# OpenDriveLab/ST-P3

Measured on AMD Instinct MI355X. Metric: BEV samples/sec (6-cam x 3-frame fwd+bwd), higher is better.
Workload: dtype bf16 convs / f32 voxel pool; 1 GPU; BASELINE configs[2]: batch=4/GPU, 6-cam 224x480, T=3, full STP3 fwd+bwd with segmentation + pedestrian + hdmap + depth CE + instance centerness/offset + flow losses, grad-clip 5, Adam; EfficientNet-B4, D=48, C=64, BEV 200x200; global_batch=4, parallelism=dp1, launch=hipgraph

## Files before the change

include/stp3_hip.h:

```cpp
#ifndef STP3_HIP_H
#define STP3_HIP_H

#include <stddef.h>
#include <stdint.h>

#ifdef __cplusplus
extern "C" {
#endif

#define STP3_OK          0
#define STP3_EINVAL   (-10001)
#define STP3_EUNSUP   (-10002)
#define STP3_ENOSPACE (-10003)

#define STP3_DTYPE_F32  0
#define STP3_DTYPE_BF16 1

typedef struct stp3_lift_dims {
    int32_t B, T, N;
    int32_t D, fH, fW;
    int32_t C;
    int32_t X, Y, Z;
} stp3_lift_dims;

// ... 123 lines not shown
int stp3_bn_bwd_train(const stp3_bn_dims* dims, const void* dy, const void* x, const float* sbias,
                      const void* res, const float* oscale, const float* mean, const float* invstd,
                      const float* gamma, const float* beta, void* workspace, size_t workspace_bytes,
                      float* sum_buf, void* dx, void* dres, void* stream);

int stp3_bn_dsbias(int32_t N, int32_t C, int32_t rows, const float* sample_sums, const float* gsums, double count,
                   const float* gamma, const float* invstd, float* dsbias, void* stream);
int stp3_sum_n(int32_t n, int64_t numel, int32_t dtype, const void* const* src, void* y, void* stream);
int stp3_sum_n_plane(int32_t n, int64_t numel, int32_t dtype, const void* const* src, const void* plane, int64_t per_sample,
                     int32_t C, void* y, void* stream);

int stp3_linear_fwd(int32_t M, int32_t K, int32_t N, const float* x, const float* w, int32_t ldw, const float* b, float* y,
                    void* stream);
int stp3_linear_bwd(int32_t M, int32_t K, int32_t N, const float* dy, const float* x, const float* w, int32_t ldw, float* dx,
                    float* dw, int32_t lddw, float* db, void* stream);

typedef struct stp3_conv_dims {
    int32_t N, H, W, Cin;
    int32_t Ho, Wo, Cout;
    int32_t KH, KW, stride;
    int32_t pad_h, pad_w, dil_h, dil_w;
    int32_t ldx, ldy;
    int32_t out_dtype, has_bias;
} stp3_conv_dims;

int stp3_conv2d_fwd_workspace(const stp3_conv_dims* dims, size_t* bytes);
int stp3_conv2d_fwd(const stp3_conv_dims* dims, const void* x, const void* w, const float* bias, void* y,
                    float* sums, void* workspace, size_t workspace_bytes, void* stream);

int stp3_conv2d_fwd_stats(const stp3_conv_dims* dims, const void* x, const void* w, float* sums, void* workspace,
                          size_t workspace_bytes, void* stream);
int stp3_conv2d_fwd_bnact(const stp3_conv_dims* dims, const void* x, const void* w, const float* coef, int32_t act, void* y,
                          void* stream);
int stp3_conv2d_bn_bwd_reduce(const stp3_conv_dims* dims, const void* x, const void* w, const void* dz, int32_t ldz,
                              const float* coef, int32_t act, float* sums, void* workspace, size_t workspace_bytes,
                              void* stream);
int stp3_conv2d_bn_bwd_apply(const stp3_conv_dims* dims, const void* x, const void* w, const void* dz, int32_t ldz,
                             const float* coef, int32_t act, const float* gsums, double count, void* dy, void* stream);
int stp3_conv2d_bn_bwd_apply_dx(const stp3_conv_dims* dims, const void* x, const void* w, const void* dz, int32_t ldz,
                                const float* coef, int32_t act, const float* gsums, double count, void* dy, void* dx,
                                int32_t lddx, const void* add, int32_t ldadd, void* stream);

int stp3_conv2d_fwd_add(const stp3_conv_dims* dims, const void* x, const void* w, const float* bias, const void* add,
                        int32_t ldadd, void* y, void* stream);

int stp3_conv2d_wgrad_workspace(const stp3_conv_dims* dims, size_t* bytes);
int stp3_conv2d_wgrad(const stp3_conv_dims* dims, const void* dy, const void* x, float* dw, void* workspace,
                      size_t workspace_bytes, void* stream);

#define STP3_WGRAD_BATCH_MAX 96
typedef struct stp3_wgrad_job {
    const void* partials;
    float* dw;
    int64_t numel;
    int32_t splits;
    int32_t reserved;
} stp3_wgrad_job;
int stp3_conv2d_wgrad_partials(const stp3_conv_dims* dims, const void* dy, const void* x, const float* pre_coef,
                               int32_t pre_act, void* partials, size_t partials_bytes, int32_t* splits, void* stream);
int stp3_conv2d_wgrad_reduce_batch(int32_t n, const stp3_wgrad_job* jobs, void* stream);

int stp3_conv2d_fwd_pre(const stp3_conv_dims* dims, const void* x, const void* w, const float* bias, const float* pre_coef,
                        int32_t pre_act, void* y, void* stream);
int stp3_conv2d_wgrad_pre(const stp3_conv_dims* dims, const void* dy, const void* x, const float* pre_coef, int32_t pre_act,
                          float* dw, void* workspace, size_t workspace_bytes, void* stream);

// ... 405 lines not shown
```

st-p3_amd/csrc/stp3_conv.hip:

```cpp
#include <hip/hip_runtime.h>
#include <stdint.h>
#include <stdlib.h>
#include <string.h>

#include "stp3_cdna.h"
#include "stp3_hip.h"

namespace {

typedef __attribute__((ext_vector_type(8))) __bf16 bf16x8;
typedef __attribute__((ext_vector_type(4))) float f32x4;
typedef __attribute__((ext_vector_type(16))) float f32x16;

struct ConvDims {
    int N, H, W, Cin, Ho, Wo, Cout;
    int KH, KW, stride, pad_h, pad_w, dil_h, dil_w;
    int ldx, ldy;
    int out_f32, has_bias;
    int M;
    int kchunks;
    int Ktot;
};

union Frag {
    uint4 u;
    bf16x8 v;
};

__device__ __forceinline__ float bf2f(uint32_t b) { return __uint_as_float(b << 16); }

constexpr int kBM = 128;
constexpr int kBK = 64;

__device__ __attribute__((aligned(16))) uint4 g_zero16 = {0u, 0u, 0u, 0u};
typedef stp3_u32x4 u32x4;

// ... 775 lines not shown
                if (!stat_partial) continue;
            }
            const uint32_t gds[4] = {g[s].x, g[s].y, g[s].z, g[s].w};
            uint32_t ow[4];
            if (MODE == kModeAffine) epi8<MODE>(wds, gds, kc[s], ep.act, s1[s], s2[s], ow, ep.res ? ep.res_mode : STP3_RES_NONE);
            else epi8<MODE>(wds, gds, kc[s], ep.act, s1[s], s2[s], ow);
            if (MODE == kModeBnAct || MODE == kModeBwdApply || MODE == kModeAffine)
                *reinterpret_cast<uint4*>(y + (size_t)m * d.ldy + ch[s]) = make_uint4(ow[0], ow[1], ow[2], ow[3]);
        }
#pragma unroll
        for (int ks = 0; ks < KMAX; ++ks) cur[ks] = nxt[ks];
    }
    if (kSums) {
        if (!stat_partial) return;
        float* mine = red + (wave * 64 + lane) * 33;
#pragma unroll
        for (int s = 0; s < 2; ++s)
#pragma unroll
            for (int r = 0; r < 8; ++r) {
                mine[s * 8 + r] = s1[s][r >> 1][r & 1];
                mine[16 + s * 8 + r] = s2[s][r >> 1][r & 1];
            }
        __builtin_amdgcn_fence(__ATOMIC_RELEASE, "wavefront");
        __builtin_amdgcn_wave_barrier();
        const int idx = lane & 31;
        float tot = 0.f;
        for (int p = 0; p < 32; ++p) tot += red[(wave * 64 + h * 32 + p) * 33 + idx];
        const int k = idx >> 4, sp = (idx >> 3) & 1, r = idx & 7;
        const int c = cb * 32 + 16 * sp + 8 * h + r;
        if (live && c < d.Cout) stat_partial[((size_t)group * 2 + k) * d.Cout + c] = tot;
    }
}

__global__ __launch_bounds__(256) void colsum_kernel(int parts, int width, const float* __restrict__ partial,
                                                     float* __restrict__ out) {
    __shared__ double red[256];
    const int cl = threadIdx.x & 63, rl = threadIdx.x >> 6;
    const int col = blockIdx.x * 64 + cl;
    const int r0 = blockIdx.y * 256, r1 = min(r0 + 256, parts);
    double s0 = 0.0, s1 = 0.0, s2 = 0.0, s3 = 0.0;
    if (col < width) {
        int p = r0 + rl;
        for (; p + 12 < r1; p += 16) {
            const float a = partial[(size_t)p * width + col], b = partial[(size_t)(p + 4) * width + col];
            const float c = partial[(size_t)(p + 8) * width + col], e = partial[(size_t)(p + 12) * width + col];
            s0 += (double)a; s1 += (double)b; s2 += (double)c; s3 += (double)e;
        }
        for (; p < r1; p += 4) s0 += (double)partial[(size_t)p * width + col];
    }
    red[threadIdx.x] = (s0 + s1) + (s2 + s3);
    __syncthreads();
    if (rl == 0 && col < width)
        out[(size_t)blockIdx.y * width + col] = (float)(red[cl] + red[64 + cl] + red[128 + cl] + red[192 + cl]);
}

inline void launch_colsum(hipStream_t s, int parts, int width, float* partial, float* sums) {
    const int wx = (width + 63) / 64;
    if (parts <= 256) {
        hipLaunchKernelGGL(colsum_kernel, dim3(wx, 1), dim3(256), 0, s, parts, width, (const float*)partial, sums);
        return;
    }
    const int l1 = (parts + 255) / 256;
    float* mid = partial + (size_t)parts * width;
    hipLaunchKernelGGL(colsum_kernel, dim3(wx, l1), dim3(256), 0, s, parts, width, (const float*)partial, mid);
    hipLaunchKernelGGL(colsum_kernel, dim3(wx, 1), dim3(256), 0, s, l1 > 256 ? 256 : l1, width, (const float*)mid, sums);
}


template <int T>
__device__ __forceinline__ int wg_piece(int m, int p) {
    const int sw = T == 64 ? ((m >> 1) & 1) << 2 : (m & 3) << 2;
    return m * (T * 2) + ((p ^ sw) << 4);
}

union FragTr {
    stp3_s16x4 h[2];
    bf16x8 v;
};

template <int TCO, int TCI, bool BUF = false, int PRE = kPreNone>
__global__ __launch_bounds__(256) void conv2d_wgrad_kernel(ConvDims d, int tiles_ci, int ksteps_per_block, int tap_fold,
                                                           int xcd_chunks, const uint16_t* __restrict__ dy,
                                                           const uint16_t* __restrict__ x,
                                                           float* __restrict__ partial, const float* __restrict__ pre = nullptr) {
    constexpr int TA = TCO / 64, TB = TCI / 64;
    constexpr int kImgA = kBK * TCO * 2;
    constexpr int kStage = kBK * (TCO + TCI) * 2;
    constexpr int PA = TCO / 8, PB = TCI / 8;
    constexpr int NA = TCO / 32, NB = TCI / 32;
    constexpr int RA = 256 / PA, RB = 256 / PB;
    extern __shared__ __attribute__((aligned(16))) uint8_t smem[];
    const int tid = threadIdx.x;
    const int lane = tid & 63;
    const int wave = __builtin_amdgcn_readfirstlane(tid >> 6);
    const int wa = wave >> 1, wb = wave & 1;
    int bx = blockIdx.x, by = blockIdx.y, bz = blockIdx.z;
    if (xcd_chunks) {
        const int lin = xcd_order(bx + (int)gridDim.x * (by + (int)gridDim.y * bz), (int)(gridDim.x * gridDim.y * gridDim.z));
// ... 410 lines not shown
    int ngroups = resident * 4 / cblocks;
    if (ngroups > (int)gx) ngroups = (int)gx;
    if (ngroups > ntiles) ngroups = ntiles;
    if (ngroups < 1) ngroups = 1;
    *parts = ngroups;
    const unsigned nwg = (unsigned)(((int64_t)ngroups * cblocks + 3) / 4);
    hipLaunchKernelGGL((pointwise_direct_kernel<KMAX, MODE>), dim3(nwg), dim3(256), 0, s, d, ksteps, cblocks, ngroups,
                       (const uint16_t*)x, (const uint16_t*)w, (uint16_t*)y, partial, ep);
    return STP3_OK;
}

template <int KMAX>
int pointwise_direct_launch_mode(int mode, const ConvDims& d, int ksteps, unsigned gx, int* parts, const void* x, const void* w,
                                 void* y, float* partial, const EpiArgs& ep, hipStream_t s) {
    switch (mode) {
        case kModePlain: return pointwise_direct_launch_one<KMAX, kModePlain>(d, ksteps, gx, parts, x, w, y, partial, ep, s);
        case kModeStats: return pointwise_direct_launch_one<KMAX, kModeStats>(d, ksteps, gx, parts, x, w, y, partial, ep, s);
        case kModeBnAct: return pointwise_direct_launch_one<KMAX, kModeBnAct>(d, ksteps, gx, parts, x, w, y, partial, ep, s);
        case kModeAffine: return pointwise_direct_launch_one<KMAX, kModeAffine>(d, ksteps, gx, parts, x, w, y, partial, ep, s);
        case kModeBwdReduce: return pointwise_direct_launch_one<KMAX, kModeBwdReduce>(d, ksteps, gx, parts, x, w, y, partial, ep, s);
        default: return pointwise_direct_launch_one<KMAX, kModeBwdApply>(d, ksteps, gx, parts, x, w, y, partial, ep, s);
    }
}

constexpr int kPointwiseMaxCin = 128;

bool pointwise_applies(const stp3_conv_dims* p, const void* y) {
    return p->KH == 1 && p->KW == 1 && p->stride == 1 && p->pad_h == 0 && p->pad_w == 0 && p->H == p->Ho && p->W == p->Wo &&
           p->Cin <= kPointwiseMaxCin && p->Cout >= 64 && !p->has_bias && p->out_dtype == STP3_DTYPE_BF16 &&
           p->Cout % 8 == 0 && p->ldy % 8 == 0 && !((uintptr_t)y & 15);
}

int pointwise_run(const ConvDims& d, const void* x, const void* w, void* y, float* sums, float* partial, unsigned gx,
                  hipStream_t s, int mode, const EpiArgs& ep) {
    const int ksteps = (d.Cin + 15) / 16;
    int rc, parts;
    const bool rows_small = (d.Cout == 144 || d.Cout == 192) && ksteps <= 2;
    const bool rows_lines = d.Cout % 64 == 0;
    if ((rows_small || rows_lines) && d.ldy % 8 == 0 && (!mode_bwd(mode) || ep.ldz % 8 == 0)) {
        const int pp = rows_small ? d.Cout / 8 : (d.Cout % 128 == 0 ? 16 : 8), nt = (pp + 3) / 4;
        const int tiles_co = d.Cout / (pp * 8);
        if (ep.dx && !(rows_small && mode == kModeBwdApply && d.Cin <= 32)) return STP3_EUNSUP;
        const size_t lds = (size_t)nt * 32 * (ksteps * 16 + 8) * 2 + (size_t)4 * 32 * (nt * 32 + 8) * 2 +
                           (ep.dx ? (size_t)32 * (nt * 32 + 8) * 2 : 0);
        unsigned per_cu = (unsigned)((160 * 1024) / lds);
        if (per_cu > 3) per_cu = 3;
        unsigned groups = (256 * per_cu + tiles_co - 1) / tiles_co;
        if (groups > gx) groups = gx;
        parts = (int)groups;
        const unsigned nwg = groups * (unsigned)tiles_co;
        if (pp == 18) rc = pointwise_rows_launch_mode<18, 2>(mode, d, ksteps, tiles_co, nwg, lds, x, w, y, partial, ep, s);
        else if (pp == 24) rc = pointwise_rows_launch_mode<24, 2>(mode, d, ksteps, tiles_co, nwg, lds, x, w, y, partial, ep, s);
        else if (pp == 8) rc = pointwise_rows_launch_mode<8, 8>(mode, d, ksteps, tiles_co, nwg, lds, x, w, y, partial, ep, s);
        else if (ksteps <= 4) rc = pointwise_rows_launch_mode<16, 4>(mode, d, ksteps, tiles_co, nwg, lds, x, w, y, partial, ep, s);
        else rc = pointwise_rows_launch_mode<16, 8>(mode, d, ksteps, tiles_co, nwg, lds, x, w, y, partial, ep, s);
    } else {
        if (ep.dx) return STP3_EUNSUP;
        if (ksteps <= 2) rc = pointwise_direct_launch_mode<2>(mode, d, ksteps, gx, &parts, x, w, y, partial, ep, s);
        else if (ksteps <= 4) rc = pointwise_direct_launch_mode<4>(mode, d, ksteps, gx, &parts, x, w, y, partial, ep, s);
        else rc = pointwise_direct_launch_mode<8>(mode, d, ksteps, gx, &parts, x, w, y, partial, ep, s);
    }
    if (rc) return rc;
    if (sums) launch_colsum(s, parts, 2 * d.Cout, partial, sums);
    return status();
}

int igemm_run(const stp3_conv_dims* p, const void* x, const void* w, const float* bias, void* y, float* sums, void* workspace,
              size_t workspace_bytes, void* stream, int mode, int act, EpiArgs ep) {
    if (!p || !x || !w || (mode != kModeStats && mode != kModeBwdReduce && !y)) return STP3_EINVAL;
    if (p->N <= 0 || p->H <= 0 || p->W <= 0 || p->Cin <= 0 || p->Cout <= 0 || p->Ho <= 0 || p->Wo <= 0 || p->KH <= 0 ||
        p->KW <= 0 || p->stride <= 0 || p->dil_h <= 0 || p->dil_w <= 0 || p->pad_h < 0 || p->pad_w < 0)
        return STP3_EINVAL;
    if (p->has_bias && !bias) return STP3_EINVAL;
    if (p->Cin % 8 || p->ldx % 8 || p->ldx < p->Cin || p->ldy < p->Cout) return STP3_EUNSUP;
    if (((uintptr_t)x & 15) || ((uintptr_t)w & 15)) return STP3_EUNSUP;
    if (p->out_dtype != STP3_DTYPE_BF16 && p->out_dtype != STP3_DTYPE_F32) return STP3_EUNSUP;
    if (y && ((uintptr_t)y & (p->out_dtype == STP3_DTYPE_F32 ? 3 : 1))) return STP3_EUNSUP;
    if ((sums || mode != kModePlain) && p->out_dtype != STP3_DTYPE_BF16) return STP3_EUNSUP;
    if (mode != kModePlain) {
        if ((p->has_bias && mode != kModeAffine) || p->Cout % 8 || p->ldy % 8 || (y && ((uintptr_t)y & 15))) return STP3_EUNSUP;
        if (mode >= kModeBnAct && !ep.coef) return STP3_EINVAL;
        if (mode == kModeAffine && ep.res && (ep.ldres % 8 || ep.ldres < p->Cout || ((uintptr_t)ep.res & 15))) return STP3_EUNSUP;
        if (mode_bwd(mode) && (!ep.dz || ep.ldz % 8 || ep.ldz < p->Cout || ((uintptr_t)ep.dz & 15))) return STP3_EUNSUP;
        if (mode == kModeBwdApply && !ep.gsums) return STP3_EINVAL;
        if ((mode == kModeStats || mode == kModeBwdReduce) && !sums) return STP3_EINVAL;
    }
    const int64_t M = (int64_t)p->N * p->Ho * p->Wo;
    if (M >= (1LL << 31) || (int64_t)p->N * p->H * p->W >= (1LL << 31)) return STP3_EUNSUP;
    ConvDims d;
    d.N = p->N; d.H = p->H; d.W = p->W; d.Cin = p->Cin; d.Ho = p->Ho; d.Wo = p->Wo; d.Cout = p->Cout;
    d.KH = p->KH; d.KW = p->KW; d.stride = p->stride; d.pad_h = p->pad_h; d.pad_w = p->pad_w;
    d.dil_h = p->dil_h; d.dil_w = p->dil_w; d.ldx = p->ldx; d.ldy = p->ldy;
    d.out_f32 = p->out_dtype == STP3_DTYPE_F32; d.has_bias = p->has_bias;
    d.M = (int)M; d.kchunks = (p->Cin + 31) / 32; d.Ktot = p->KH * p->KW * p->Cin;
    const unsigned gx = (unsigned)((M + kBM - 1) / kBM);
    hipStream_t s = (hipStream_t)stream;
    float* partial = nullptr;
    if (sums) {
        if (gx > 65536) return STP3_EUNSUP;
        if (!workspace || workspace_bytes < ((size_t)gx + (gx + 255) / 256) * 2 * p->Cout * sizeof(float)) return STP3_ENOSPACE;
        partial = (float*)workspace;
    }
    if (y && ((uintptr_t)y & 15)) return STP3_EUNSUP;
    if (ep.dx) {
        if (!pointwise_applies(p, y) || ep.lddx % 4 || ep.lddx < p->Cin || ((uintptr_t)ep.dx & 7) ||
            (ep.add && (ep.ldadd % 4 || ep.ldadd < p->Cin || ((uintptr_t)ep.add & 7))))
            return STP3_EUNSUP;
        ep.act = act;
        return pointwise_run(d, x, w, y, sums, partial, gx, s, mode, ep);
    }
    if (ep.pre) {
        if (mode != kModePlain || sums || ep.add || p->KH != 1 || p->KW != 1 || p->stride != 1 || p->pad_h || p->pad_w ||
            p->H != p->Ho || p->W != p->Wo || p->Cin > 4096)
            return STP3_EUNSUP;
        if (!((size_t)d.N * d.H * d.W * d.ldx * 2 < (1ull << 31) && (size_t)d.Cout * d.Ktot * 2 < (1ull << 31))) return STP3_EUNSUP;
    } else if (ep.add) {
        if (mode != kModePlain || d.out_f32 || p->Cout % 8 || p->ldy % 8 || ep.ldadd % 8 || ep.ldadd < p->Cout ||
            ((uintptr_t)ep.add & 15) || ((uintptr_t)y & 15))
            return STP3_EUNSUP;
    } else if (pointwise_applies(p, y)) {
        if (ep.sbias) return STP3_EUNSUP;
        ep.act = act;
        return pointwise_run(d, x, w, y, sums, partial, gx, s, mode, ep);
    }
    const int steps = (d.Ktot + kBK - 1) / kBK;
    const bool wide = p->Cout > 64 && steps > 2 && (int64_t)gx * ((p->Cout + 127) / 128) >= 512;
    const int bn = wide ? 128 : 64;
    size_t lds = igemm_lds(bn, steps, d.out_f32 != 0);
    if (mode == kModeBwdReduce) {
        const size_t need = (size_t)2 * kBM * (bn + 8) * 2 + 512 * sizeof(float);
        if (need > lds) lds = need;
    }
    const int tiles_co = (p->Cout + bn - 1) / bn;
    if ((int64_t)gx * tiles_co >= (1LL << 31)) return STP3_EUNSUP;
    const dim3 grid(gx * (unsigned)tiles_co);
    int rc;
    if (ep.pre) {
        ep.pre_off = (int)((lds + 15) / 16 * 16);
        lds = (size_t)ep.pre_off + (size_t)2 * steps * kBK * sizeof(float);
        if (act == STP3_ACT_RELU)
            rc = wide ? igemm_launch_pre<128, kPreRelu>(d, grid, lds, tiles_co, x, w, bias, y, ep, s)
                      : igemm_launch_pre<64, kPreRelu>(d, grid, lds, tiles_co, x, w, bias, y, ep, s);
        else
            rc = wide ? igemm_launch_pre<128, kPreAffine>(d, grid, lds, tiles_co, x, w, bias, y, ep, s)
                      : igemm_launch_pre<64, kPreAffine>(d, grid, lds, tiles_co, x, w, bias, y, ep, s);
        return rc ? rc : status();
    }
#define STP3_IGEMM_MODE(MODE)                                                                                                \
    rc = wide ? igemm_launch_act<128, MODE>(act, d, grid, lds, tiles_co, x, w, bias, y, partial, ep, s)                       \
              : igemm_launch_act<64, MODE>(act, d, grid, lds, tiles_co, x, w, bias, y, partial, ep, s)
    switch (mode) {
        case kModePlain: STP3_IGEMM_MODE(kModePlain); break;
        case kModeStats: STP3_IGEMM_MODE(kModeStats); break;
        case kModeBnAct: STP3_IGEMM_MODE(kModeBnAct); break;
        case kModeAffine: STP3_IGEMM_MODE(kModeAffine); break;
        case kModeBwdReduce: STP3_IGEMM_MODE(kModeBwdReduce); break;
        default: STP3_IGEMM_MODE(kModeBwdApply); break;
    }
#undef STP3_IGEMM_MODE
    if (rc) return rc;
    if (sums) launch_colsum(s, (int)gx, 2 * p->Cout, partial, sums);
    return status();
}

}

extern "C" {

int stp3_conv2d_fwd(const stp3_conv_dims* p, const void* x, const void* w, const float* bias, void* y, float* sums,
                    void* workspace, size_t workspace_bytes, void* stream) {
    return igemm_run(p, x, w, bias, y, sums, workspace, workspace_bytes, stream, kModePlain, STP3_ACT_NONE, EpiArgs());
}

int stp3_conv2d_fwd_pre(const stp3_conv_dims* p, const void* x, const void* w, const float* bias, const float* pre_coef,
                        int32_t pre_act, void* y, void* stream) {
    if (!pre_coef || (pre_act != STP3_ACT_NONE && pre_act != STP3_ACT_RELU)) return STP3_EINVAL;
    EpiArgs ep = EpiArgs();
    ep.pre = pre_coef;
    return igemm_run(p, x, w, bias, y, nullptr, nullptr, 0, stream, kModePlain, pre_act, ep);
}

int stp3_conv2d_fwd_add(const stp3_conv_dims* p, const void* x, const void* w, const float* bias, const void* add, int32_t ldadd,
                        void* y, void* stream) {
    if (!add) return STP3_EINVAL;
    EpiArgs ep = EpiArgs();
    ep.add = (const uint16_t*)add;
    ep.ldadd = ldadd;
    return igemm_run(p, x, w, bias, y, nullptr, nullptr, 0, stream, kModePlain, STP3_ACT_NONE, ep);
}

int stp3_conv2d_fwd_stats(const stp3_conv_dims* p, const void* x, const void* w, float* sums, void* workspace,
                          size_t workspace_bytes, void* stream) {
    return igemm_run(p, x, w, nullptr, nullptr, sums, workspace, workspace_bytes, stream, kModeStats, STP3_ACT_NONE, EpiArgs());
}

int stp3_conv2d_fwd_bnact(const stp3_conv_dims* p, const void* x, const void* w, const float* coef, int32_t act, void* y,
                          void* stream) {
    EpiArgs ep = EpiArgs();
    ep.coef = coef;
    return igemm_run(p, x, w, nullptr, y, nullptr, nullptr, 0, stream, kModeBnAct, act, ep);
}

int stp3_conv2d_fwd_affine(const stp3_conv_dims* p, const void* x, const void* w, const float* bias, const float* coef,
                           const float* sbias, int32_t channels, int32_t act, const void* res, int32_t ldres, int32_t res_mode,
                           void* y, void* stream) {
    if (!p || !coef) return STP3_EINVAL;
    if (act != STP3_ACT_NONE && act != STP3_ACT_RELU && act != STP3_ACT_SWISH) return STP3_EINVAL;
    if (res_mode != STP3_RES_NONE && res_mode != STP3_RES_BEFORE_ACT && res_mode != STP3_RES_AFTER_ACT) return STP3_EINVAL;
    if ((res_mode != STP3_RES_NONE) != (res != nullptr)) return STP3_EINVAL;
    if (channels <= 0 || channels > p->Cout) return STP3_EINVAL;
    if (p->Cout != (channels + 7) / 8 * 8) return STP3_EUNSUP;
    EpiArgs ep = EpiArgs();
    ep.coef = coef; ep.res = (const uint16_t*)res; ep.ldres = ldres; ep.res_mode = res_mode; ep.cvalid = channels;
    ep.sbias = sbias; ep.hw = p->Ho > 0 && p->Wo > 0 ? p->Ho * p->Wo : 1;
    return igemm_run(p, x, w, bias, y, nullptr, nullptr, 0, stream, kModeAffine, act, ep);
}

int stp3_conv2d_bn_bwd_reduce(const stp3_conv_dims* p, const void* x, const void* w, const void* dz, int32_t ldz,
                              const float* coef, int32_t act, float* sums, void* workspace, size_t workspace_bytes,
                              void* stream) {
    EpiArgs ep = EpiArgs();
    ep.coef = coef; ep.dz = (const uint16_t*)dz; ep.ldz = ldz;
    return igemm_run(p, x, w, nullptr, nullptr, sums, workspace, workspace_bytes, stream, kModeBwdReduce, act, ep);
}

int stp3_conv2d_bn_bwd_apply(const stp3_conv_dims* p, const void* x, const void* w, const void* dz, int32_t ldz,
// ... 157 lines not shown
```

st-p3_amd/stp3_amd/_lib.py:

```python
import ctypes
import os

from . import profiling

_HERE = os.path.dirname(os.path.abspath(__file__))
LIB_PATH = os.path.join(_HERE, 'libstp3hip.so')

c_void_p = ctypes.c_void_p
c_int = ctypes.c_int
c_int32 = ctypes.c_int32
c_float = ctypes.c_float
c_size_t = ctypes.c_size_t


class LiftDims(ctypes.Structure):
    _fields_ = [(k, ctypes.c_int32) for k in ('B', 'T', 'N', 'D', 'fH', 'fW', 'C', 'X', 'Y', 'Z')]

    @property
    def BT(self):
        return self.B * self.T

    @property
    def NPIX(self):
        return self.N * self.fH * self.fW
# ... 228 lines not shown
                                    c_float, c_void_p, c_size_t, c_void_p, c_void_p, c_void_p]),
    'stp3_gru_reset_cat_fwd': (c_int, [_GRU_P, c_void_p, c_void_p, c_void_p, c_void_p]),
    'stp3_gru_output_fwd': (c_int, [_GRU_P, c_void_p, c_void_p, c_void_p, c_void_p, c_void_p]),
    'stp3_gru_output_bwd': (c_int, [_GRU_P, c_void_p, ctypes.c_int32, c_void_p, c_void_p, c_void_p, c_void_p, c_void_p, c_void_p]),
    'stp3_gru_reset_cat_bwd': (c_int, [_GRU_P, c_void_p, ctypes.c_int32, c_void_p, c_void_p, c_void_p, c_void_p, c_void_p, c_void_p]),
    'stp3_layernorm_fwd': (c_int, [_LN_P, c_void_p, c_void_p, c_void_p, c_void_p, c_void_p]),
    'stp3_layernorm_bwd_workspace': (c_int, [_LN_P, ctypes.POINTER(c_size_t)]),
    'stp3_layernorm_bwd': (c_int, [_LN_P] + [c_void_p] * 8 + [c_size_t, c_void_p]),
    'stp3_dwconv2d_fwd': (c_int, [_DW_P, c_void_p, c_void_p, c_void_p, c_void_p]),
    'stp3_dwconv2d_fwd_bias': (c_int, [_DW_P, c_void_p, c_void_p, c_void_p, c_void_p, c_void_p]),
    'stp3_dwconv2d_bwd_data': (c_int, [_DW_P, c_void_p, c_void_p, c_void_p, c_void_p]),
    'stp3_dwconv2d_bwd_weight_workspace': (c_int, [_DW_P, ctypes.POINTER(c_size_t)]),
    'stp3_dwconv2d_bwd_weight': (c_int, [_DW_P, c_void_p, c_void_p, c_void_p, c_void_p, c_size_t, c_void_p]),
    'stp3_dwconv2d_bwd_weight_oihw': (c_int, [_DW_P, c_void_p, c_void_p, c_void_p, c_void_p, c_size_t, c_void_p]),
    'stp3_bn_workspace_bytes': (c_int, [_BN_P, ctypes.POINTER(c_size_t)]),
    'stp3_bn_stats': (c_int, [_BN_P, c_void_p, c_void_p, c_void_p, c_size_t, c_void_p, c_void_p]),
    'stp3_bn_apply_fwd': (c_int, [_BN_P] + [c_void_p] * 5 + [c_double, c_void_p, c_void_p, c_float, c_float]
                          + [c_void_p] * 6),
    'stp3_bn_bwd_reduce': (c_int, [_BN_P] + [c_void_p] * 10 + [c_size_t, c_void_p, c_void_p, c_void_p]),
    'stp3_bn_apply_bwd': (c_int, [_BN_P] + [c_void_p] * 10 + [c_double, c_void_p, c_void_p, c_void_p]),
    'stp3_bn_fwd_train': (c_int, [_BN_P] + [c_void_p] * 6 + [c_float, c_float] + [c_void_p] * 4 + [c_size_t, c_void_p,
                                                                                                 c_void_p]),
    'stp3_bn_bwd_train': (c_int, [_BN_P] + [c_void_p] * 10 + [c_size_t] + [c_void_p] * 4),
    'stp3_bn_dsbias': (c_int, [c_int32, c_int32, c_int32, c_void_p, c_void_p, c_double, c_void_p, c_void_p, c_void_p, c_void_p]),
    'stp3_sum_n': (c_int, [c_int32, ctypes.c_int64, c_int32, c_void_p, c_void_p, c_void_p]),
    'stp3_linear_fwd': (c_int, [c_int32, c_int32, c_int32, c_void_p, c_void_p, c_int32, c_void_p, c_void_p, c_void_p]),
    'stp3_linear_bwd': (c_int, [c_int32, c_int32, c_int32, c_void_p, c_void_p, c_void_p, c_int32, c_void_p, c_void_p, c_int32, c_void_p,
                                c_void_p]),
    'stp3_sum_n_plane': (c_int, [c_int32, ctypes.c_int64, c_int32, c_void_p, c_void_p, ctypes.c_int64, c_int32, c_void_p, c_void_p]),
    'stp3_conv2d_fwd_workspace': (c_int, [ctypes.POINTER(ConvDims), ctypes.POINTER(c_size_t)]),
    'stp3_conv2d_fwd': (c_int, [ctypes.POINTER(ConvDims)] + [c_void_p] * 6 + [c_size_t, c_void_p]),
    'stp3_conv2d_fwd_add': (c_int, [ctypes.POINTER(ConvDims), c_void_p, c_void_p, c_void_p, c_void_p, c_int32, c_void_p, c_void_p]),
    'stp3_conv2d_fwd_stats': (c_int, [ctypes.POINTER(ConvDims), c_void_p, c_void_p, c_void_p, c_void_p, c_size_t, c_void_p]),
    'stp3_conv2d_fwd_bnact': (c_int, [ctypes.POINTER(ConvDims), c_void_p, c_void_p, c_void_p, c_int32, c_void_p, c_void_p]),
    'stp3_conv2d_bn_bwd_reduce': (c_int, [ctypes.POINTER(ConvDims), c_void_p, c_void_p, c_void_p, c_int32, c_void_p, c_int32,
                                          c_void_p, c_void_p, c_size_t, c_void_p]),
    'stp3_conv2d_bn_bwd_apply': (c_int, [ctypes.POINTER(ConvDims), c_void_p, c_void_p, c_void_p, c_int32, c_void_p, c_int32,
                                         c_void_p, c_double, c_void_p, c_void_p]),
    'stp3_se_workspace_bytes': (c_int, [ctypes.POINTER(SeDims), ctypes.POINTER(c_size_t)]),
    'stp3_se_pool': (c_int, [ctypes.POINTER(SeDims), c_void_p, c_void_p, c_void_p, c_size_t, c_void_p, c_void_p]),
    'stp3_se_scale': (c_int, [ctypes.POINTER(SeDims), c_void_p, c_void_p, c_void_p, c_void_p, c_void_p]),
    'stp3_conv2d_bn_bwd_apply_dx': (c_int, [ctypes.POINTER(ConvDims), c_void_p, c_void_p, c_void_p, c_int32, c_void_p, c_int32, c_void_p,
                                            ctypes.c_double, c_void_p, c_void_p, c_int32, c_void_p, c_int32, c_void_p]),
    'stp3_conv2d_wgrad_workspace': (c_int, [ctypes.POINTER(ConvDims), ctypes.POINTER(c_size_t)]),
    'stp3_conv2d_wgrad': (c_int, [ctypes.POINTER(ConvDims), c_void_p, c_void_p, c_void_p, c_void_p, c_size_t, c_void_p]),
    'stp3_conv2d_wgrad_partials': (c_int, [ctypes.POINTER(ConvDims), c_void_p, c_void_p, c_void_p, c_int32, c_void_p, c_size_t,
                                           ctypes.POINTER(c_int32), c_void_p]),
    'stp3_conv2d_fwd_pre': (c_int, [ctypes.POINTER(ConvDims), c_void_p, c_void_p, c_void_p, c_void_p, c_int32, c_void_p, c_void_p]),
    'stp3_conv2d_wgrad_pre': (c_int, [ctypes.POINTER(ConvDims), c_void_p, c_void_p, c_void_p, c_int32, c_void_p, c_void_p, c_size_t,
                                      c_void_p]),
    'stp3_conv2d_wgrad_reduce_batch': (c_int, [c_int32, ctypes.POINTER(WgradJob), c_void_p]),
    'stp3_conv2d_prep_weights': (c_int, [c_void_p, c_int32, ctypes.c_int64, c_void_p]),
    'stp3_conv2d_scatter_weight_grads': (c_int, [c_void_p, c_int32, ctypes.c_int64, c_void_p]),
    'stp3_se_mlp_fwd': (c_int, [c_void_p] * 9),
    'stp3_se_mlp_bwd': (c_int, [c_void_p] * 15),
    'stp3_optim_workspace_bytes': (c_int, [ctypes.c_int64, ctypes.POINTER(c_size_t)]),
    'stp3_optim_clip_adam': (c_int, [c_void_p, c_int32, ctypes.c_int64] + [c_float] * 6 + [c_void_p, c_void_p, c_size_t,
                                                                                          c_void_p]),
    'stp3_causal_pair_fwd': (c_int, [ctypes.POINTER(PairDims), c_void_p, c_void_p, c_void_p]),
    'stp3_causal_pair_bwd': (c_int, [ctypes.POINTER(PairDims), c_void_p, c_void_p, c_void_p]),
    'stp3_upsample_bilinear_fwd': (c_int, [ctypes.POINTER(UpsampleDims), c_void_p, c_void_p, c_void_p]),
    'stp3_upsample_bilinear_bwd': (c_int, [ctypes.POINTER(UpsampleDims), c_void_p, c_void_p, c_void_p]),
    'stp3_dwconv2d_fwd_stats_workspace': (c_int, [_DW_P, ctypes.POINTER(c_size_t)]),
    'stp3_dwconv2d_fwd_stats': (c_int, [_DW_P, c_void_p, c_void_p, c_void_p, c_void_p, c_void_p, c_size_t, c_void_p]),
    'stp3_bn_finalize': (c_int, [c_void_p, c_int32, c_double, c_void_p, c_void_p, c_float, c_float, c_void_p, c_void_p,
                                 c_void_p, c_void_p]),
# ... 118 lines not shown
```

st-p3_amd/stp3_amd/ops_fused.py:

```python
import ctypes
import os

import torch

from . import _lib, ops, scratch
from ._lib import check

_SE_MLP = True


def conv2d_v2(x, wb, bias, stride, pad, dil, sums_ptr=None):
    return ops._conv2d_launch(x, wb, bias, stride, pad, dil, torch.bfloat16, sums_ptr=sums_ptr)


class _ConvBnAct(torch.autograd.Function):
    @staticmethod
    def forward(ctx, x, weight, cbias, gamma, beta, res, running_mean, running_var, momentum, eps, act, res_mode,
                stride, pad, dil, group, oscale=None, out_slot=None, res_carrier=None, skip_carrier=None):
        return ops.drive_exchange(_ConvBnAct.forward_steps(ctx, x, weight, cbias, gamma, beta, res, running_mean,
                                                           running_var, momentum, eps, act, res_mode, stride, pad, dil,
                                                           group, oscale, out_slot, res_carrier, skip_carrier), group)

    @staticmethod
    def backward(ctx, dy):
# ... 103 lines not shown
        skip_grad = None if skip_carrier is None else skip_carrier.take()
        cout, cin, kh, kw = wb.shape
        dx = dw = dcb = None
        bpad = (dil[0] * (kh - 1) - pad[0], dil[1] * (kw - 1) - pad[1])
        need_dx = ctx.needs_input_grad[0]
        hip_dx = need_dx and cout % 8 == 0 and bpad[0] >= 0 and bpad[1] >= 0
        if hip_dx:
            dx = ops.conv2d_data_grad(dconv, wb, ctx.weight_ref, x.shape, stride, pad, dil, add=skip_grad)
            skip_grad = None
        need_dw = ctx.needs_input_grad[1]
        need_db = has_cbias and ctx.needs_input_grad[2]
        hip_dw = need_dw and cin % 8 == 0 and cout % 8 == 0
        if hip_dw:
            dw = ops._conv2d_wgrad(dconv, x, (cout, cin, kh, kw), stride, pad, dil, leaf=ctx.weight_ref).to(wdt)
            if need_db:
                dcb = ops.channel_sums(dconv).to(cbdt)
        mask = [need_dx and not hip_dx, need_dw and not hip_dw, need_db and not hip_dw]
        if any(mask):
            xd = x if x.is_contiguous(memory_format=torch.channels_last) else x.contiguous(memory_format=torch.channels_last)
            gx, gw, gb = torch.ops.aten.convolution_backward(dconv, xd, wb, [cout] if has_cbias else None, [stride, stride],
                                                             list(pad), list(dil), False, [0, 0], 1, mask)
            if mask[0]:
                dx = gx
            if mask[1]:
                dw = gw.to(wdt)
            if mask[2]:
                dcb = gb.to(cbdt)
        if skip_grad is not None:
            dx = skip_grad if dx is None else dx + skip_grad.to(dx.dtype)
        return (dx, dw, dcb, dgamma, dbeta, dres) + (None,) * 14


EXPAND_DGRAD_IN_APPLY = True


class _PointwiseBnAct(torch.autograd.Function):

    @staticmethod
    def forward(ctx, x, weight, gamma, beta, running_mean, running_var, momentum, eps, act, group, skip_carrier=None):
        return ops.drive_exchange(_PointwiseBnAct.forward_steps(ctx, x, weight, gamma, beta, running_mean, running_var,
                                                                momentum, eps, act, group, skip_carrier), group)

    @staticmethod
    def backward(ctx, dz):
        return ops.drive_exchange(_PointwiseBnAct.backward_steps(ctx, dz), ctx.cfg[3])

    @staticmethod
    def forward_steps(ctx, x, weight, gamma, beta, running_mean, running_var, momentum, eps, act, group, skip_carrier=None):
        ops._need_gpu(x, weight)
        ctx.skip_carrier = skip_carrier
        if x.dtype != torch.bfloat16:
            x = x.to(torch.bfloat16)
        wb, _ = ops._bf16_weights(weight)
        cout, cin = wb.shape[:2]
        n, _, h, w = x.shape
        x, ldx = ops._rows_view(x)
        dev = x.device
        lib = _lib.lib()
        dims = _lib.ConvDims(n, h, w, cin, h, w, cout, 1, 1, 1, 0, 0, 1, 1, ldx, cout, _lib.DTYPE_BF16, 0)
        need = ctypes.c_size_t()
        check(lib.stp3_conv2d_fwd_workspace(ctypes.byref(dims), ctypes.byref(need)), 'stp3_conv2d_fwd_workspace')
        ws = scratch.get('fused', need.value, dev, floor=32 << 20)
        stat = torch.empty(6 * cout, dtype=torch.float32, device=dev)
        stream = ops._stream_handle()
        check(lib.stp3_conv2d_fwd_stats(ctypes.byref(dims), x.data_ptr(), wb.data_ptr(), stat.data_ptr(), ws.data_ptr(),
                                        need.value, stream), 'stp3_conv2d_fwd_stats')
        count = float(n * h * w)
        world, exchange = ops.replicas(group)
        if exchange:
            yield stat[:2 * cout]
            count *= world
        g32, b32 = ops._f32(gamma), ops._f32(beta)
        coef = stat[2 * cout:]
        check(lib.stp3_bn_finalize(stat.data_ptr(), cout, count, ops._opt_ptr(g32), ops._opt_ptr(b32), eps, momentum,
                                   ops._opt_ptr(running_mean), ops._opt_ptr(running_var), coef.data_ptr(), stream),
              'stp3_bn_finalize')
        y = torch.empty((n, cout, h, w), dtype=torch.bfloat16, device=dev, memory_format=torch.channels_last)
        check(lib.stp3_conv2d_fwd_bnact(ctypes.byref(dims), x.data_ptr(), wb.data_ptr(), coef.data_ptr(), int(act), y.data_ptr(),
                                        stream), 'stp3_conv2d_fwd_bnact')
        ctx.save_for_backward(x, wb, coef)
        ctx.cfg = (dims, count, exchange, group, int(act), need.value)
        ctx.weight_ref = ops.note_weight_use(weight)
        ctx.weight_stamp = ops.weight_stamp(weight)
        ctx.dtypes = (weight.dtype, None if gamma is None else gamma.dtype, None if beta is None else beta.dtype)
        return y

    @staticmethod
    def backward_steps(ctx, dz):
        x, wb, coef = ctx.saved_tensors
        ops.check_weight_stamp(ctx.weight_ref, ctx.weight_stamp, 'pointwise_bn_act backward')
        dims, count, exchange, group, act, ws_bytes = ctx.cfg
        wdt, gdt, bdt = ctx.dtypes
        cout, cin = wb.shape[:2]
        dev = x.device
        lib = _lib.lib()
        if dz.dtype != torch.bfloat16:
            dz = dz.to(torch.bfloat16)
        dz, ldz = ops._rows_view(dz)
        if ldz % 8 or dz.data_ptr() % 16:
            dz, ldz = dz.contiguous(memory_format=torch.channels_last), cout
        ws = scratch.get('fused', ws_bytes, dev, floor=32 << 20)
        stream = ops._stream_handle()
        lsums = torch.empty(2, cout, dtype=torch.float32, device=dev)
        check(lib.stp3_conv2d_bn_bwd_reduce(ctypes.byref(dims), x.data_ptr(), wb.data_ptr(), dz.data_ptr(), ldz, coef.data_ptr(),
                                            act, lsums.data_ptr(), ws.data_ptr(), ws_bytes, stream), 'stp3_conv2d_bn_bwd_reduce')
        gsums = lsums
        if exchange:
            gsums = lsums.clone()
            yield gsums
# ... 577 lines not shown
```

Baseline: 112.6 samples/s.

## Rewrite column-sum reduction and fuse BN finalize into stats reduction

Replaces the column-sum kernel with a templated version that gives each thread four columns, uses vector loads, picks a wider lane count, and splits into one or two levels with a larger chunk. The intermediate level is stored in double. The new kernel can optionally run the BatchNorm finalize (coefficients and running-stat update) in its last level, which would drop a separate finalize launch. That fused path sits behind a flag that is off by default, so only the rewritten reduction runs; the new reduction touches every stats-producing conv.

Measured after the change: 113.1 samples/s (median of 6 runs). No clear change (+0.4%).

```diff
diff --git a/include/stp3_hip.h b/include/stp3_hip.h
--- a/include/stp3_hip.h
+++ b/include/stp3_hip.h
@@ -179,6 +179,10 @@
                           size_t workspace_bytes, void* stream);
 int stp3_conv2d_fwd_bnact(const stp3_conv_dims* dims, const void* x, const void* w, const float* coef, int32_t act, void* y,
                           void* stream);
+int stp3_conv2d_fwd_stats_bn(const stp3_conv_dims* dims, const void* x, const void* w, float* sums, double count,
+                             const float* gamma, const float* beta, float eps, float momentum, float* running_mean,
+                             float* running_var, float* coef, void* workspace, size_t workspace_bytes, void* stream);
+int stp3_conv2d_stats_reduce(int32_t parts, int32_t C, float* partial, float* sums, void* stream);
 int stp3_conv2d_bn_bwd_reduce(const stp3_conv_dims* dims, const void* x, const void* w, const void* dz, int32_t ldz,
                               const float* coef, int32_t act, float* sums, void* workspace, size_t workspace_bytes,
                               void* stream);
diff --git a/st-p3_amd/csrc/stp3_conv.hip b/st-p3_amd/csrc/stp3_conv.hip
--- a/st-p3_amd/csrc/stp3_conv.hip
+++ b/st-p3_amd/csrc/stp3_conv.hip
@@ -2,6 +2,7 @@
 #include <stdint.h>
 #include <stdlib.h>
 #include <string.h>
+#include <type_traits>
 
 #include "stp3_cdna.h"
 #include "stp3_hip.h"
@@ -843,38 +844,121 @@
     }
 }
 
-__global__ __launch_bounds__(256) void colsum_kernel(int parts, int width, const float* __restrict__ partial,
-                                                     float* __restrict__ out) {
-    __shared__ double red[256];
-    const int cl = threadIdx.x & 63, rl = threadIdx.x >> 6;
-    const int col = blockIdx.x * 64 + cl;
-    const int r0 = blockIdx.y * 256, r1 = min(r0 + 256, parts);
-    double s0 = 0.0, s1 = 0.0, s2 = 0.0, s3 = 0.0;
-    if (col < width) {
-        int p = r0 + rl;
-        for (; p + 12 < r1; p += 16) {
-            const float a = partial[(size_t)p * width + col], b = partial[(size_t)(p + 4) * width + col];
-            const float c = partial[(size_t)(p + 8) * width + col], e = partial[(size_t)(p + 12) * width + col];
-            s0 += (double)a; s1 += (double)b; s2 += (double)c; s3 += (double)e;
-        }
-        for (; p < r1; p += 4) s0 += (double)partial[(size_t)p * width + col];
-    }
-    red[threadIdx.x] = (s0 + s1) + (s2 + s3);
+struct BnFin {
+    float inv_count, unbias, eps, momentum;
+    const float* gamma;
+    const float* beta;
+    float* running_mean;
+    float* running_var;
+    float* coef;
+};
+
+constexpr int kColsumMaxLanes = 128, kColsumPieces = 8;
+template <typename TIn, typename TOut>
+__global__ __launch_bounds__(kColsumPieces * kColsumMaxLanes) void colsum_kernel(int parts, int C, int L, int chunk, int vec,
+                                                                                  const TIn* __restrict__ partial,
+                                                                                  TOut* __restrict__ out, BnFin f) {
+    __shared__ double red[4][kColsumPieces * kColsumMaxLanes];
+    constexpr int G = kColsumPieces;
+    const int tid = threadIdx.x;
+    const int g = tid % G, lane = tid / G;
+    const int width = 2 * C;
+    const int c0 = blockIdx.x * 16 + (g & 3) * 4;
+    const int col0 = f.coef ? (g >> 2) * C + c0 : blockIdx.x * 32 + g * 4;
+    const int ncol = f.coef ? C - c0 : width - col0;
+    const int r0 = blockIdx.y * chunk, r1 = min(r0 + chunk, parts);
+    double s[4][4];
+#pragma unroll
+    for (int i = 0; i < 4; ++i)
+#pragma unroll
+        for (int j = 0; j < 4; ++j) s[i][j] = 0.0;
+    if (ncol > 0) {
+        const TIn* src = partial + col0;
+        auto row = [&](int p, TIn v[4]) {
+            const TIn* q = src + (size_t)p * width;
+            if constexpr (std::is_same<TIn, float>::value) {
+                if (vec) {
+                    const float4 t = *reinterpret_cast<const float4*>(q);
+                    v[0] = t.x; v[1] = t.y; v[2] = t.z; v[3] = t.w;
+                    return;
+                }
+            }
+#pragma unroll
+            for (int j = 0; j < 4; ++j) v[j] = j < ncol ? q[j] : (TIn)0;
+        };
+        int p = r0 + lane;
+        for (; p + 3 * L < r1; p += 4 * L) {
+            TIn v[4][4];
+#pragma unroll
+            for (int i = 0; i < 4; ++i) row(p + i * L, v[i]);
+#pragma unroll
+            for (int i = 0; i < 4; ++i)
+#pragma unroll
+                for (int j = 0; j < 4; ++j) s[i][j] += (double)v[i][j];
+        }
+        for (; p < r1; p += L) {
+            TIn v[4];
+            row(p, v);
+#pragma unroll
+            for (int j = 0; j < 4; ++j) s[0][j] += (double)v[j];
+        }
+    }
+#pragma unroll
+    for (int j = 0; j < 4; ++j) red[j][tid] = (s[0][j] + s[1][j]) + (s[2][j] + s[3][j]);
     __syncthreads();
-    if (rl == 0 && col < width)
-        out[(size_t)blockIdx.y * width + col] = (float)(red[cl] + red[64 + cl] + red[128 + cl] + red[192 + cl]);
-}
-
-inline void launch_colsum(hipStream_t s, int parts, int width, float* partial, float* sums) {
-    const int wx = (width + 63) / 64;
-    if (parts <= 256) {
-        hipLaunchKernelGGL(colsum_kernel, dim3(wx, 1), dim3(256), 0, s, parts, width, (const float*)partial, sums);
+    for (int st = L / 2; st > 0; st >>= 1) {
+        if (lane < st) {
+#pragma unroll
+            for (int j = 0; j < 4; ++j) red[j][tid] += red[j][tid + st * G];
+        }
+        __syncthreads();
+    }
+    if (lane != 0 || ncol <= 0) return;
+#pragma unroll
+    for (int j = 0; j < 4; ++j)
+        if (j < ncol) out[(size_t)blockIdx.y * width + col0 + j] = (TOut)red[j][tid];
+    if (!f.coef || g >= 4) return;
+    for (int j = 0; j < 4; ++j) {
+        const int c = c0 + j;
+        if (c >= C) break;
+        const float sum = (float)red[j][tid], sq = (float)red[j][tid + 4];
+        const float mean = sum * f.inv_count;
+        const float var = fmaxf(sq * f.inv_count - mean * mean, 0.f);
+        const float invstd = 1.0f / sqrtf(var + f.eps);
+        const float scale = (f.gamma ? f.gamma[c] : 1.f) * invstd;
+        f.coef[c] = scale;
+        f.coef[C + c] = (f.beta ? f.beta[c] : 0.f) - mean * scale;
+        f.coef[2 * C + c] = mean;
+        f.coef[3 * C + c] = invstd;
+        if (f.running_mean) {
+            f.running_mean[c] = (1.f - f.momentum) * f.running_mean[c] + f.momentum * mean;
+            f.running_var[c] = (1.f - f.momentum) * f.running_var[c] + f.momentum * var * f.unbias;
+        }
+    }
+}
+
+template <typename TIn, typename TOut>
+inline void launch_colsum_level(hipStream_t s, int rows, int chunk, int C, const TIn* in, TOut* out, const BnFin* fin) {
+    int L = 32;
+    while (L < kColsumMaxLanes && 4 * L < chunk) L *= 2;
+    const int vec = !((uintptr_t)in & 15) && (fin ? C % 4 == 0 : C % 2 == 0);
+    BnFin f = BnFin();
+    if (fin) f = *fin;
+    const int nx = fin ? (C + 15) / 16 : (2 * C + 31) / 32;
+    hipLaunchKernelGGL((colsum_kernel<TIn, TOut>), dim3(nx, (rows + chunk - 1) / chunk), dim3(kColsumPieces * L), 0, s, rows, C, L,
+                       chunk, vec, in, out, f);
+}
+
+constexpr int kColsumOneLevel = 2048, kColsumChunk = 1024;
+inline void launch_colsum(hipStream_t s, int parts, int C, float* partial, float* sums, const BnFin* fin = nullptr) {
+    if (parts <= kColsumOneLevel) {
+        launch_colsum_level<float, float>(s, parts, parts, C, partial, sums, fin);
         return;
     }
-    const int l1 = (parts + 255) / 256;
-    float* mid = partial + (size_t)parts * width;
-    hipLaunchKernelGGL(colsum_kernel, dim3(wx, l1), dim3(256), 0, s, parts, width, (const float*)partial, mid);
-    hipLaunchKernelGGL(colsum_kernel, dim3(wx, 1), dim3(256), 0, s, l1 > 256 ? 256 : l1, width, (const float*)mid, sums);
+    double* mid = reinterpret_cast<double*>(((uintptr_t)(partial + (size_t)parts * 2 * C) + 7) & ~(uintptr_t)7);
+    launch_colsum_level<float, double>(s, parts, kColsumChunk, C, partial, mid, nullptr);
+    const int l1 = (parts + kColsumChunk - 1) / kColsumChunk;
+    launch_colsum_level<double, float>(s, l1, l1, C, mid, sums, fin);
 }
 
 
@@ -1351,7 +1435,7 @@
 }
 
 int pointwise_run(const ConvDims& d, const void* x, const void* w, void* y, float* sums, float* partial, unsigned gx,
-                  hipStream_t s, int mode, const EpiArgs& ep) {
+                  hipStream_t s, int mode, const EpiArgs& ep, const BnFin* fin = nullptr) {
     const int ksteps = (d.Cin + 15) / 16;
     int rc, parts;
     const bool rows_small = (d.Cout == 144 || d.Cout == 192) && ksteps <= 2;
@@ -1380,12 +1464,12 @@
         else rc = pointwise_direct_launch_mode<8>(mode, d, ksteps, gx, &parts, x, w, y, partial, ep, s);
     }
     if (rc) return rc;
-    if (sums) launch_colsum(s, parts, 2 * d.Cout, partial, sums);
+    if (sums) launch_colsum(s, parts, d.Cout, partial, sums, fin);
     return status();
 }
 
 int igemm_run(const stp3_conv_dims* p, const void* x, const void* w, const float* bias, void* y, float* sums, void* workspace,
-              size_t workspace_bytes, void* stream, int mode, int act, EpiArgs ep) {
+              size_t workspace_bytes, void* stream, int mode, int act, EpiArgs ep, const BnFin* fin = nullptr) {
     if (!p || !x || !w || (mode != kModeStats && mode != kModeBwdReduce && !y)) return STP3_EINVAL;
     if (p->N <= 0 || p->H <= 0 || p->W <= 0 || p->Cin <= 0 || p->Cout <= 0 || p->Ho <= 0 || p->Wo <= 0 || p->KH <= 0 ||
         p->KW <= 0 || p->stride <= 0 || p->dil_h <= 0 || p->dil_w <= 0 || p->pad_h < 0 || p->pad_w < 0)
@@ -1426,7 +1510,7 @@
             (ep.add && (ep.ldadd % 4 || ep.ldadd < p->Cin || ((uintptr_t)ep.add & 7))))
             return STP3_EUNSUP;
         ep.act = act;
-        return pointwise_run(d, x, w, y, sums, partial, gx, s, mode, ep);
+        return pointwise_run(d, x, w, y, sums, partial, gx, s, mode, ep, fin);
     }
     if (ep.pre) {
         if (mode != kModePlain || sums || ep.add || p->KH != 1 || p->KW != 1 || p->stride != 1 || p->pad_h || p->pad_w ||
@@ -1440,7 +1524,7 @@
     } else if (pointwise_applies(p, y)) {
         if (ep.sbias) return STP3_EUNSUP;
         ep.act = act;
-        return pointwise_run(d, x, w, y, sums, partial, gx, s, mode, ep);
+        return pointwise_run(d, x, w, y, sums, partial, gx, s, mode, ep, fin);
     }
     const int steps = (d.Ktot + kBK - 1) / kBK;
     const bool wide = p->Cout > 64 && steps > 2 && (int64_t)gx * ((p->Cout + 127) / 128) >= 512;
@@ -1478,7 +1562,7 @@
     }
 #undef STP3_IGEMM_MODE
     if (rc) return rc;
-    if (sums) launch_colsum(s, (int)gx, 2 * p->Cout, partial, sums);
+    if (sums) launch_colsum(s, (int)gx, p->Cout, partial, sums, fin);
     return status();
 }
 
@@ -1511,6 +1595,26 @@
 int stp3_conv2d_fwd_stats(const stp3_conv_dims* p, const void* x, const void* w, float* sums, void* workspace,
                           size_t workspace_bytes, void* stream) {
     return igemm_run(p, x, w, nullptr, nullptr, sums, workspace, workspace_bytes, stream, kModeStats, STP3_ACT_NONE, EpiArgs());
+}
+
+int stp3_conv2d_fwd_stats_bn(const stp3_conv_dims* p, const void* x, const void* w, float* sums, double count, const float* gamma,
+                             const float* beta, float eps, float momentum, float* running_mean, float* running_var, float* coef,
+                             void* workspace, size_t workspace_bytes, void* stream) {
+    if (!coef || !(count >= 1.0)) return STP3_EINVAL;
+    if ((running_mean == nullptr) != (running_var == nullptr)) return STP3_EINVAL;
+    BnFin fin;
+    fin.inv_count = (float)(1.0 / count);
+    fin.unbias = count > 1.0 ? (float)(count / (count - 1.0)) : 1.f;
+    fin.eps = eps; fin.momentum = momentum; fin.gamma = gamma; fin.beta = beta;
+    fin.running_mean = running_mean; fin.running_var = running_var; fin.coef = coef;
+    return igemm_run(p, x, w, nullptr, nullptr, sums, workspace, workspace_bytes, stream, kModeStats, STP3_ACT_NONE, EpiArgs(), &fin);
+}
+
+int stp3_conv2d_stats_reduce(int32_t parts, int32_t C, float* partial, float* sums, void* stream) {
+    if (!partial || !sums || parts <= 0 || C <= 0) return STP3_EINVAL;
+    if (parts > 65536) return STP3_EUNSUP;
+    launch_colsum((hipStream_t)stream, parts, C, partial, sums);
+    return status();
 }
 
 int stp3_conv2d_fwd_bnact(const stp3_conv_dims* p, const void* x, const void* w, const float* coef, int32_t act, void* y,
diff --git a/st-p3_amd/stp3_amd/_lib.py b/st-p3_amd/stp3_amd/_lib.py
--- a/st-p3_amd/stp3_amd/_lib.py
+++ b/st-p3_amd/stp3_amd/_lib.py
@@ -284,6 +284,9 @@
     'stp3_conv2d_fwd': (c_int, [ctypes.POINTER(ConvDims)] + [c_void_p] * 6 + [c_size_t, c_void_p]),
     'stp3_conv2d_fwd_add': (c_int, [ctypes.POINTER(ConvDims), c_void_p, c_void_p, c_void_p, c_void_p, c_int32, c_void_p, c_void_p]),
     'stp3_conv2d_fwd_stats': (c_int, [ctypes.POINTER(ConvDims), c_void_p, c_void_p, c_void_p, c_void_p, c_size_t, c_void_p]),
+    'stp3_conv2d_fwd_stats_bn': (c_int, [ctypes.POINTER(ConvDims), c_void_p, c_void_p, c_void_p, c_double, c_void_p, c_void_p, c_float,
+                                         c_float, c_void_p, c_void_p, c_void_p, c_void_p, c_size_t, c_void_p]),
+    'stp3_conv2d_stats_reduce': (c_int, [c_int32, c_int32, c_void_p, c_void_p, c_void_p]),
     'stp3_conv2d_fwd_bnact': (c_int, [ctypes.POINTER(ConvDims), c_void_p, c_void_p, c_void_p, c_int32, c_void_p, c_void_p]),
     'stp3_conv2d_bn_bwd_reduce': (c_int, [ctypes.POINTER(ConvDims), c_void_p, c_void_p, c_void_p, c_int32, c_void_p, c_int32,
                                           c_void_p, c_void_p, c_size_t, c_void_p]),
diff --git a/st-p3_amd/stp3_amd/ops_fused.py b/st-p3_amd/stp3_amd/ops_fused.py
--- a/st-p3_amd/stp3_amd/ops_fused.py
+++ b/st-p3_amd/stp3_amd/ops_fused.py
@@ -159,6 +159,7 @@
 
 
 EXPAND_DGRAD_IN_APPLY = True
+EXPAND_STATS_BN = False
 
 
 class _PointwiseBnAct(torch.autograd.Function):
@@ -190,18 +191,24 @@
         ws = scratch.get('fused', need.value, dev, floor=32 << 20)
         stat = torch.empty(6 * cout, dtype=torch.float32, device=dev)
         stream = ops._stream_handle()
-        check(lib.stp3_conv2d_fwd_stats(ctypes.byref(dims), x.data_ptr(), wb.data_ptr(), stat.data_ptr(), ws.data_ptr(),
-                                        need.value, stream), 'stp3_conv2d_fwd_stats')
         count = float(n * h * w)
         world, exchange = ops.replicas(group)
-        if exchange:
-            yield stat[:2 * cout]
-            count *= world
         g32, b32 = ops._f32(gamma), ops._f32(beta)
         coef = stat[2 * cout:]
-        check(lib.stp3_bn_finalize(stat.data_ptr(), cout, count, ops._opt_ptr(g32), ops._opt_ptr(b32), eps, momentum,
-                                   ops._opt_ptr(running_mean), ops._opt_ptr(running_var), coef.data_ptr(), stream),
-              'stp3_bn_finalize')
+        if EXPAND_STATS_BN and not exchange:
+            check(lib.stp3_conv2d_fwd_stats_bn(ctypes.byref(dims), x.data_ptr(), wb.data_ptr(), stat.data_ptr(), count,
+                                               ops._opt_ptr(g32), ops._opt_ptr(b32), eps, momentum, ops._opt_ptr(running_mean),
+                                               ops._opt_ptr(running_var), coef.data_ptr(), ws.data_ptr(), need.value, stream),
+                  'stp3_conv2d_fwd_stats_bn')
+        else:
+            check(lib.stp3_conv2d_fwd_stats(ctypes.byref(dims), x.data_ptr(), wb.data_ptr(), stat.data_ptr(), ws.data_ptr(),
+                                            need.value, stream), 'stp3_conv2d_fwd_stats')
+            if exchange:
+                yield stat[:2 * cout]
+                count *= world
+            check(lib.stp3_bn_finalize(stat.data_ptr(), cout, count, ops._opt_ptr(g32), ops._opt_ptr(b32), eps, momentum,
+                                       ops._opt_ptr(running_mean), ops._opt_ptr(running_var), coef.data_ptr(), stream),
+                  'stp3_bn_finalize')
         y = torch.empty((n, cout, h, w), dtype=torch.bfloat16, device=dev, memory_format=torch.channels_last)
         check(lib.stp3_conv2d_fwd_bnact(ctypes.byref(dims), x.data_ptr(), wb.data_ptr(), coef.data_ptr(), int(act), y.data_ptr(),
                                         stream), 'stp3_conv2d_fwd_bnact')
```
